# davelee2804/MiMSEM

Hardware: AMD Instinct MI355X
Metric: element operator-applies/sec (higher is better)
Workload: dtype f64; 1 GPU; Umat (B1) matrix-free apply, p=3 24x24x6 cubed sphere x 30 levels (BASELINE config 4 grid); order=3, elements=3456, levels=30, patches_per_gpu=24, form=wave-level fused (k_apply_wave + k_wave_perim)

## Files before the change

include/mimsem_hip.h:

```cpp
#ifndef MIMSEM_HIP_H
#define MIMSEM_HIP_H

#ifdef __cplusplus
extern "C" {
#endif

#define MIMSEM_ABI_VERSION 1

enum {
    MIMSEM_OK = 0,
    MIMSEM_ERR_ARG = -1,
    MIMSEM_ERR_UNSUPPORTED = -2,
    MIMSEM_ERR_HIP = -3,
    MIMSEM_ERR_STATE = -4,
    MIMSEM_ERR_SINGULAR = -5
};

typedef struct mimsem_ctx mimsem_ctx;

typedef struct mimsem_mesh_desc {
    int elOrd;
    int quadOrd;
    int nEl;
    int nk;
// ... 46 lines not shown
const char* mimsem_strerror(int code);
const char* mimsem_last_hip_error(void);
int  mimsem_device_count(void);

int  mimsem_ctx_create(const mimsem_mesh_desc* desc, int device, mimsem_ctx** out);
void mimsem_ctx_destroy(mimsem_ctx* ctx);
int  mimsem_ctx_set_stream(mimsem_ctx* ctx, void* hip_stream);
int  mimsem_ctx_sync(mimsem_ctx* ctx);
int  mimsem_ctx_set_levels(mimsem_ctx* ctx, const double* thick, const double* thickInv);
long long mimsem_ctx_workspace_bytes(const mimsem_ctx* ctx);
int  mimsem_op_level_chunk(const mimsem_ctx* ctx, int nlev);
int  mimsem_op_wave_stats(const mimsem_ctx* ctx, int nlev, int out[5]);
int  mimsem_ctx_set_wave_split(mimsem_ctx* ctx, int part_levels, int order);
int  mimsem_ctx_set_wave_balance(mimsem_ctx* ctx, int ncu, int wgs_per_cu);
long long mimsem_ctx_wave_balance_launches(const mimsem_ctx* ctx);
#define MIMSEM_PART_ALL      0
#define MIMSEM_PART_BOUNDARY 1
#define MIMSEM_PART_INTERIOR 2
int  mimsem_ctx_set_halo_slots(mimsem_ctx* ctx, int form, const int* slots, int n);
int  mimsem_op_apply_part(mimsem_ctx* ctx, int op, int geom_lev0, int nlev, double scale, unsigned flags,
                          const double* f, long long f_stride, const double* x, long long x_stride,
                          double* y, long long y_stride, double alpha, int part);
int  mimsem_op_apply_part_reset(mimsem_ctx* ctx);
int  mimsem_ctx_set_profiling(mimsem_ctx* ctx, int on);
int  mimsem_ctx_profile_read(mimsem_ctx* ctx, double* ms_pass1, double* ms_pass2, long long* launches);

int  mimsem_ctx_use_own_stream(mimsem_ctx* ctx);
int  mimsem_malloc(void** dev, long long bytes);
int  mimsem_free(void* dev);
int  mimsem_memcpy_h2d(mimsem_ctx* ctx, void* dev, const void* host, long long bytes);
// ... 309 lines not shown
```

mimsem_amd/_lib.py:

```python
import ctypes as C
import os
import subprocess

_HERE = os.path.dirname(os.path.abspath(__file__))
LIB_PATH = os.environ.get("MIMSEM_LIB") or os.path.join(_HERE, "libmimsem_hip.so")

c_dp = C.c_void_p
c_ll = C.c_longlong


class MeshDesc(C.Structure):
    _fields_ = [("elOrd", C.c_int), ("quadOrd", C.c_int), ("nEl", C.c_int), ("nk", C.c_int),
                ("n0", C.c_int), ("n1", C.c_int), ("n2", C.c_int),
                ("inds0", C.c_void_p), ("inds1x", C.c_void_p), ("inds1y", C.c_void_p), ("inds2", C.c_void_p),
                ("det", C.c_void_p), ("J", C.c_void_p), ("thick", C.c_void_p), ("thickInv", C.c_void_p),
                ("indsq", C.c_void_p), ("nq", C.c_int)]


class MimsemError(RuntimeError):
    pass


_SIGS = {
    "mimsem_abi_version": (C.c_int, []),
# ... 1 lines not shown
    "mimsem_strerror": (C.c_char_p, [C.c_int]),
    "mimsem_last_hip_error": (C.c_char_p, []),
    "mimsem_device_count": (C.c_int, []),
    "mimsem_ctx_create": (C.c_int, [C.POINTER(MeshDesc), C.c_int, C.POINTER(C.c_void_p)]),
    "mimsem_ctx_destroy": (None, [C.c_void_p]),
    "mimsem_ctx_set_stream": (C.c_int, [C.c_void_p, C.c_void_p]),
    "mimsem_ctx_use_own_stream": (C.c_int, [C.c_void_p]),
    "mimsem_ctx_sync": (C.c_int, [C.c_void_p]),
    "mimsem_ctx_set_levels": (C.c_int, [C.c_void_p, C.c_void_p, C.c_void_p]),
    "mimsem_ctx_workspace_bytes": (c_ll, [C.c_void_p]),
    "mimsem_op_level_chunk": (C.c_int, [C.c_void_p, C.c_int]),
    "mimsem_op_wave_stats": (C.c_int, [C.c_void_p, C.c_int, C.POINTER(C.c_int)]),
    "mimsem_ctx_set_wave_split": (C.c_int, [C.c_void_p, C.c_int, C.c_int]),
    "mimsem_ctx_set_wave_balance": (C.c_int, [C.c_void_p, C.c_int, C.c_int]),
    "mimsem_ctx_wave_balance_launches": (c_ll, [C.c_void_p]),
    "mimsem_ctx_set_halo_slots": (C.c_int, [C.c_void_p, C.c_int, C.c_void_p, C.c_int]),
    "mimsem_op_apply_part": (C.c_int, [C.c_void_p, C.c_int, C.c_int, C.c_int, C.c_double, C.c_uint, c_dp, c_ll, c_dp, c_ll, c_dp, c_ll, C.c_double, C.c_int]),
    "mimsem_ctx_set_profiling": (C.c_int, [C.c_void_p, C.c_int]),
    "mimsem_ctx_profile_read": (C.c_int, [C.c_void_p, C.POINTER(C.c_double), C.POINTER(C.c_double), C.POINTER(c_ll)]),
    "mimsem_malloc": (C.c_int, [C.POINTER(C.c_void_p), c_ll]),
    "mimsem_free": (C.c_int, [C.c_void_p]),
    "mimsem_memcpy_h2d": (C.c_int, [C.c_void_p, C.c_void_p, C.c_void_p, c_ll]),
    "mimsem_memcpy_d2h": (C.c_int, [C.c_void_p, C.c_void_p, C.c_void_p, c_ll]),
    "mimsem_memset": (C.c_int, [C.c_void_p, C.c_void_p, C.c_int, c_ll]),
    "mimsem_op_apply": (C.c_int, [C.c_void_p, C.c_int, C.c_int, C.c_int, C.c_double, C.c_uint,
                                  c_dp, c_ll, c_dp, c_ll, c_dp, c_ll, C.c_double]),
    "mimsem_op_apply_levels": (C.c_int, [C.c_void_p, C.c_int, C.c_int, C.c_int, C.c_int, C.c_double, C.c_uint,
                                         c_dp, c_ll, c_dp, c_ll, c_dp, c_ll, C.c_double]),
    "mimsem_op_apply_up": (C.c_int, [C.c_void_p, C.c_int, C.c_int, C.c_int, C.c_double, C.c_double, C.c_uint,
                                     c_dp, c_ll, c_dp, c_ll, c_dp, c_ll, c_dp, c_ll, C.c_double]),
# ... 184 lines not shown
```

mimsem_amd/csrc/api.hip:

```cpp
#include <algorithm>
#include <cstdio>
#include <cstdlib>
#include <climits>
#include <cstring>
#include "ctx.hpp"
#include "wave_balance.hpp"

namespace mimsem {
thread_local std::string g_last_hip_error;
int hip_fail(hipError_t e, const char* what) {
    g_last_hip_error = std::string(what) + ": " + hipGetErrorString(e);
    return MIMSEM_ERR_HIP;
}
}

namespace {

template <class T>
int upload(T** dst, const T* src, size_t count, mimsem_ctx* c) {
    if (int rc = c->alloc((void**)dst, count*sizeof(T))) return rc;
    if (count) MIMSEM_HIP_TRY(hipMemcpy(*dst, src, count*sizeof(T), hipMemcpyHostToDevice));
    return MIMSEM_OK;
}

// ... 479 lines not shown
        };
        for (int p : owned[g]) {
            ent.push_back(int4{2*p, (int)(contrib(2*p, 0) | contrib(2*p, 1) << 16), (int)(contrib(2*p + 1, 0) | contrib(2*p + 1, 1) << 16), 0});
            W.ndirect += 2;
        }
        if (ent.empty() || ent.size() > 64) return MIMSEM_ERR_UNSUPPORTED;
        for (int t = 0; t < 64; t++) W.plan[(size_t)g*64 + t] = ent[t%ent.size()];
        W.nsides += (int)sides.size(); W.maxsides = std::max(W.maxsides, (int)sides.size());
        if (sides.size() == 4 && nxs > 0 && nys > 0) W.nfull++;
        W.mix[nxs == 2 && nys == 2 ? 0 : (nxs == 4 && nys == 0 ? 1 : (nxs == 0 && nys == 4 ? 2 : 3))]++;
        W.maxgx = std::max(W.maxgx, 16*(int)sides.size());
    }
    return MIMSEM_OK;
}

int level_chunk(const mimsem_ctx* c, int nlev) {
    const ElemSizes& es = c->es;
    const int epb = 256/(es.mp12 <= 4 ? 4 : (es.mp12 <= 16 ? 16 : (es.mp12 <= 32 ? 32 : 64)));
    const long long blocks1 = ((long long)c->nEl + epb - 1)/epb;
    long long lch = (blocks1*nlev)/(256*6);
    if (lch < 1) lch = 1;
    if (lch > nlev) lch = nlev;
    if (lch > 8) lch = 8;
    if (c->lch_override > 0) lch = std::min(c->lch_override, nlev);
    return (int)std::max(1LL, lch);
}

int wave_level_chunk(const mimsem_ctx* c, int nlev) {
    if (c->wave_lch > 0) return std::max(1, std::min(std::min(c->wave_lch, 8), nlev));
    return std::max(1, std::min(8, nlev));
// ... 158 lines not shown
    const bool own = want_own && build_wave_own(es.n, c->n1, c->nEl, es.n1e, 64/lpe, c->h_i1x.data(), c->h_i1y.data(), P, W) == MIMSEM_OK;
    WaveTables t;
    const size_t mark = c->owned.size();
    rc = [&]() -> int {
        int rc;
        if ((rc = upload(&t.lane, P.lane.data(), P.lane.size(), c))) return rc;
        if ((rc = upload(&t.plan, P.plan.data(), P.plan.size(), c))) return rc;
        std::vector<int4> rec(P.pslot.size());
        for (size_t i = 0; i < rec.size(); i++) rec[i] = int4{P.pslot[i], P.ppart[2*i], P.ppart[2*i + 1], 0};
        if ((rc = upload(&t.prec, rec.data(), rec.size(), c))) return rc;
        if ((rc = upload(&t.node, P.node.data(), P.node.size(), c))) return rc;
        if (own) {
            if ((rc = upload(&t.oplan, W.plan.data(), W.plan.size(), c))) return rc;
            if ((rc = upload(&t.gh, W.gh.data(), W.gh.size(), c))) return rc;
            if ((rc = upload(&t.gx, W.gx.data(), W.gx.size(), c))) return rc;
            if (own4 && (rc = upload(&t.gh4, W.gh4.data(), W.gh4.size(), c))) return rc;
        }
        if (P.nsing && (rc = upload(&t.sing, P.sing.data(), P.sing.size(), c))) return rc;
        if ((rc = upload(&t.fin, P.fin.data(), P.fin.size(), c))) return rc;
        if ((rc = upload(&t.sslot, P.sslot.data(), P.sslot.size(), c))) return rc;
        if (P.ntiles > 0 && (rc = upload(&t.tfin, P.tfin.data(), P.tfin.size(), c))) return rc;
        const size_t n = (size_t)std::max(P.nsides, 1)*(size_t)std::max(c->nk, 1);
        if ((rc = c->alloc((void**)&t.cnt, n*sizeof(int)))) return rc;
        MIMSEM_HIP_TRY(hipMemset(t.cnt, 0, n*sizeof(int)));
        std::vector<double> G, Rv;
        pack_wave_metric(c, P, lpe, G, Rv);
        if ((rc = upload(&t.G, G.data(), G.size(), c))) return rc;
        return upload(&t.R, Rv.data(), Rv.size(), c);
    }();
    if (rc) { while (c->owned.size() > mark) c->release(c->owned.back().first); return rc; }
    t.on = true; t.own = own; t.can_fin = P.fin_ok && want_fin; t.split = marked != nullptr;
    t.ndirect = P.ndirect; t.ngroups = P.ngroups; t.nsing = P.nsing; t.nps = P.nps; t.npart = P.npart; t.npwritten = P.npwritten; t.nsides = P.nsides;
    if (P.ntiles > 0) { t.ntiles = P.ntiles; t.ninner = P.ninner; }
    t.nbgroups = P.nbgroups; t.nbrec = P.nbrec;
    c->wv = t;
    if (const char* kind = exp_env("MIMSEM_WPART_MEM")) c->w_partmem = !strcmp(kind, "plain") ? 2 : (!strcmp(kind, "finegrained") ? 1 : 0);
    if (const char* ev = exp_env("MIMSEM_WAVE_ORDER")) c->wave_order = atoi(ev);
    if (const char* ev = exp_env("MIMSEM_WAVE_LCH")) c->wave_lch = atoi(ev);
    if (const char* ev = exp_env("MIMSEM_WAVE_CPP")) c->wave_cpp = atoi(ev);
    if (const char* ev = exp_env("MIMSEM_WAVE2")) c->wave2_mode = atoi(ev);
    if (getenv("MIMSEM_VERBOSE"))
        fprintf(stderr, "[mimsem] wave plan: %d groups of %d elements (%d on the halo boundary), %d perimeter slots (%d partials in %d sides) of %d; "
// ... 288 lines not shown
    if (g->g) (void)hipGraphDestroy(g->g);
    delete g;
}
int mimsem_ctx_sync(mimsem_ctx* c) { if (!c) return MIMSEM_ERR_ARG; MIMSEM_HIP_TRY(hipStreamSynchronize(c->stream)); return MIMSEM_OK; }
long long mimsem_ctx_workspace_bytes(const mimsem_ctx* c) { return c ? c->bytes : 0; }
int mimsem_op_level_chunk(const mimsem_ctx* c, int nlev) { return (c && nlev > 0) ? level_chunk(c, nlev) : MIMSEM_ERR_ARG; }
int mimsem_op_wave_stats(const mimsem_ctx* c, int nlev, int out[5]) {
    if (!c || !out || nlev < 1) return MIMSEM_ERR_ARG;
    for (int i = 0; i < 5; i++) out[i] = 0;
    if (!c->wv.on) return 0;
    out[0] = c->wv.ngroups; out[1] = c->wv.ndirect; out[2] = c->wv.npwritten; out[3] = c->wv.nps;
    if (c->wv.own) { out[1] = c->n1; out[2] = 0; out[3] = 0; }
    if (c->wv.own && c->es.n == 3 && c->wv.ntiles == 0 && !c->d_tIn) {
        const WaveParts wp = wave_level_parts(c, nlev, c->wv.ngroups);
        out[4] = wp.longest;
        const int nwg = c->wv.gh4 ? wave_balance_workgroups(c, nlev, c->wv.ngroups, wp) : 0;
        const mimsem_ctx::BalList* b = nwg > 0 ? wave_balance_find(c, nlev, c->wv.ngroups, nwg) : nullptr;
        if (b && b->items) out[4] = b->longest;
    }
    else { const int lch = wave_level_chunk(c, nlev); out[4] = lch*wave_chunks_per_item(c, nlev, lch, c->wv.ngroups); }
    return 1;
}

int mimsem_ctx_set_wave_split(mimsem_ctx* c, int part_levels, int order) {
    if (!c || part_levels < 0 || order < -1 || order > 3) return MIMSEM_ERR_ARG;
    if (c->is_capturing()) return MIMSEM_ERR_STATE;
    c->wave_part = part_levels;
    if (order >= 0) c->wave_order = order;
    return MIMSEM_OK;
}

int mimsem_ctx_set_wave_balance(mimsem_ctx* c, int ncu, int wgs_per_cu) {
    if (!c || ncu > (1 << 20) || (ncu >= 0 && (wgs_per_cu < 1 || wgs_per_cu > 3))) return MIMSEM_ERR_ARG;
    if (c->is_capturing()) return MIMSEM_ERR_STATE;
    c->bal_ncu = ncu < 0 ? -1 : ncu;
    if (ncu >= 0) c->bal_k = wgs_per_cu;
    return MIMSEM_OK;
}
long long mimsem_ctx_wave_balance_launches(const mimsem_ctx* c) { return c ? c->bal_launches : MIMSEM_ERR_ARG; }

int mimsem_ctx_set_levels(mimsem_ctx* c, const double* thick, const double* thickInv) {
    if (!c) return MIMSEM_ERR_ARG;
    if (c->is_capturing()) return MIMSEM_ERR_STATE;
    MIMSEM_HIP_TRY(hipStreamSynchronize(c->stream));
    const size_t cnt = (size_t)c->nk*c->nEl*c->es.mp12;
    std::vector<double> th(cnt, 1.0), ti(cnt, 1.0);
    if (thick) std::memcpy(th.data(), thick, cnt*sizeof(double));
    if (thickInv) std::memcpy(ti.data(), thickInv, cnt*sizeof(double));
    else if (thick) for (size_t i = 0; i < cnt; i++) ti[i] = 1.0/th[i];
    else if (false) {}
    if (cnt) {
        MIMSEM_HIP_TRY(hipMemcpy(c->d_th, th.data(), cnt*sizeof(double), hipMemcpyHostToDevice));
        MIMSEM_HIP_TRY(hipMemcpy(c->d_tI, ti.data(), cnt*sizeof(double), hipMemcpyHostToDevice));
    }
// ... 169 lines not shown
    return a;
}
static void basis_by_value(const mimsem_ctx* c, ElemArgs& a) {
    for (size_t k = 0; k < 20; k++) a.Etab[k] = k < c->tab.E.size() ? c->tab.E[k] : 0.0;
    for (size_t k = 0; k < 5; k++) a.Wq[k] = k < c->tab.quad.w.size() ? c->tab.quad.w[k] : 0.0;
}
static bool fits_32bit(const mimsem_ctx* c, bool nodes) {
    const long long lim = 1LL << 28;
    return (long long)c->n1 < lim && (!nodes || (long long)c->n0 < lim) && (long long)c->n2 < lim && (long long)c->nEl*c->es.mp12 < lim;
}

#ifdef MIMSEM_STAMPS
static long long* g_stamps = nullptr; static size_t g_stamp_items = 0;
static size_t stamps_begin(mimsem_ctx* c, int nlev, ElemArgs& a) {
    const size_t items = (size_t)c->wv.ngroups*std::max((nlev + a.lch - 1)/a.lch, a.wnp);
    if (!exp_env("MIMSEM_WAVE_STAMPS")) return items;
    if (items > g_stamp_items) { if (g_stamps) (void)hipFree(g_stamps); (void)hipMalloc((void**)&g_stamps, items*16*8); g_stamp_items = items; }
    (void)hipMemsetAsync(g_stamps, 0, items*16*8, c->stream);
    a.wstamps = g_stamps;
    return items;
}
static void stamps_report(mimsem_ctx* c, const ElemArgs& a, size_t items) {
    if (!a.wstamps) return;
    (void)hipStreamSynchronize(c->stream);
    std::vector<long long> h(items*16);
    (void)hipMemcpy(h.data(), g_stamps, items*16*8, hipMemcpyDeviceToHost);
    long long t0 = h[0], t1 = 0;
    for (size_t i = 0; i < items; i++) { t0 = std::min(t0, h[i*16]); t1 = std::max(t1, h[i*16 + 15]); }
    fprintf(stderr, "[stamps] items %zu lch %d  first entry -> last done: %lld ticks\n", items, a.lch, t1 - t0);
    const char* names[16] = {"entry(rel. first)", "barrier", "tables requested", "level loads issued", "batch0", "batch1", "batch2", "batch3",
                             "b4", "b5", "b6", "chunks done", "fin: stores acked", "fin: arrival counted", "fin: sides finished", "stores acked"};
    for (int k = 0; k < 16; k++) {
        std::vector<long long> v;
        for (size_t i = 0; i < items; i++) if (h[i*16 + k]) v.push_back(k == 0 ? h[i*16] - t0 : h[i*16 + k] - h[i*16]);
        if (v.empty()) continue;
        std::sort(v.begin(), v.end());
        fprintf(stderr, "[stamps] %-20s min %8lld  p10 %8lld  median %8lld  p90 %8lld  max %8lld   (ticks since the wave's entry)\n", names[k],
                v.front(), v[v.size()/10], v[v.size()/2], v[v.size()*9/10], v.back());
    }
}
#endif


static int apply_wave2(mimsem_ctx* c, const ApplyCall& k, ElemArgs& a) {
    if (int rc = c->ensure_ye(64)) return rc;
    a.wlane = c->wv.lane; a.wgroups = c->wv.ngroups; a.wG = c->wv.G; a.wR = c->wv.R;
// ... 26 lines not shown
    const int rc = launch_elem_apply(c, k.op, a);
    return rc ? rc : launch_gather_perim(c, k.nlev, c->d_ye, c->f_npart, a.accum, k.y, k.ys);
}

static int apply_wave1(mimsem_ctx* c, const ApplyCall& k, ElemArgs& a, bool splits) {
    const WaveTables& w = c->wv;
    const ElemSizes& es = c->es;
    const int nlev = k.nlev;
    const bool own = w.own && !splits && k.op == MIMSEM_OP_UMAT && es.n == 3 && !c->d_tIn && w.ntiles == 0;
    const long long prow = (own ? 0LL : (long long)w.npart) + 128;
    int g0 = 0, g1 = w.ngroups, r0 = 0, r1 = w.nps;
    if (splits && k.part == MIMSEM_PART_BOUNDARY) { g1 = w.nbgroups; r1 = w.nbrec; }
    if (splits && k.part == MIMSEM_PART_INTERIOR) { g0 = w.nbgroups; r0 = w.nbrec; }
    a.wlane = w.lane; a.wplan = own ? w.oplan : w.plan; a.wgroups = g1 - g0; a.wg0 = g0; a.wdump = own ? 0 : w.npart;
    a.wgh = own ? w.gh : nullptr; a.wgx = w.gx;
    a.wgh4 = (own && (long long)c->nEl*es.mp12 < (1LL << 27)) ? w.gh4 : nullptr;
    a.wsing = w.nsing ? w.sing : nullptr; a.wnode = w.node; a.wG = w.G; a.wR = w.R;
    if (c->d_tIn) { a.tIp = c->d_tIn; a.tps = (long long)c->n0*2; a.tnode = 1; }
    a.lch = wave_level_chunk(c, nlev);
    a.wcpp = wave_chunks_per_item(c, nlev, a.lch, g1 - g0);
    if (own) {
        const WaveParts wp = wave_level_parts(c, nlev, g1 - g0);
        a.wnp = wp.np; a.wpb = wp.pb; a.wpr = wp.pr;
        a.lch = nlev == 1 ? 1 : 8; a.wcpp = 1;
        if (const int nwg = a.wgh4 ? wave_balance_workgroups(c, nlev, g1 - g0, wp) : 0) {
            const mimsem_ctx::BalList* b = wave_balance_find(c, nlev, g1 - g0, nwg);
            if (!b && !c->is_capturing()) {
                if (int rc = wave_balance_make(c, nlev, g1 - g0, nwg, wp)) return rc;
                b = &c->bal.back();
            }
            if (b && b->items) { a.witems = b->items; a.wnitems = b->nitems; }
        }
    }
    a.swz = c->wave_order;
    if (w.ntiles > 0) {
        if (splits) return MIMSEM_ERR_STATE;
        a.wtfin = w.tfin; a.wtile = WTF;
        a.wcpp = std::min(a.wcpp, MIMSEM_WTLEV/8);
        a.swz &= ~2;
// ... 434 lines not shown
```

mimsem_amd/csrc/ctx.hpp:

```cpp
#pragma once
#include <hip/hip_runtime.h>
#include <string>
#include <utility>
#include <vector>
#include "../../include/mimsem_hip.h"
#include "basis_host.hpp"
#include <cstdlib>

constexpr int MIMSEM_RD_COUNTERS = 8;
#ifdef MIMSEM_WITH_EXPERIMENTS
constexpr bool kExperiments = true;
inline const char* exp_env(const char* name) {
    static const bool on = std::getenv("MIMSEM_EXPERIMENTS") && std::atoi(std::getenv("MIMSEM_EXPERIMENTS")) != 0;
    return on ? std::getenv(name) : nullptr;
}
#else
constexpr bool kExperiments = false;
inline const char* exp_env(const char*) { return nullptr; }
#endif

namespace mimsem {
extern thread_local std::string g_last_hip_error;
int hip_fail(hipError_t e, const char* what);
}
// ... 12 lines not shown
struct WaveTables {
    bool on = false;
    int ngroups = 0, nsing = 0, nps = 0, npart = 0, ndirect = 0;
    int npwritten = 0;
    bool can_fin = false;
    int nsides = 0;
    int4* fin = nullptr;
    int* sslot = nullptr;
    int* cnt = nullptr;
    int nbgroups = 0, nbrec = 0; bool split = false;
    int4* lane = nullptr;
    bool own = false;
    int4* oplan = nullptr;
    int4* gh = nullptr;
    int* gx = nullptr;
    int4* gh4 = nullptr;
    int4* tfin = nullptr; int ntiles = 0, ninner = 0;
    int4* plan = nullptr;
    int2* sing = nullptr;
    int* node = nullptr;
    double* G = nullptr;
    double* R = nullptr;
    int4* prec = nullptr;
};

enum class Mem { Plain, Uncached, FineGrained };

struct mimsem_ctx {
    int device = 0;
    hipStream_t stream = nullptr;
    hipStream_t cap_stream = nullptr, cap_saved = nullptr; bool cap_active = false, cap_swapped = false;
// ... 170 lines not shown
};
struct PairBlocks { int nEl, lch; const int *i1x, *i1y, *plan; const double *B, *ye; long long yes; const double* b; double* ze; long long zes; const int4* bplan; };
struct PairGather { const double* ye; long long yes; const int* plan; int nslots; GatherEpilogue g; double* x; };
int launch_sw_pair(mimsem_ctx* c, int PA, int PB, const ElemArgs& ea, const PairBlocks& ba, const PairGather& ga, const ElemArgs& eq, const PairGather& gq);
int launch_gather_epilogue(mimsem_ctx* c, int form, int nlev, const double* ye, long long ye_stride, const GatherEpilogue& g,
                           double* x, long long xs);
int launch_blocks_residual(mimsem_ctx* c, int nlev, const double* B, const double* ye, long long yes,
                           const double* b, long long bs, double* ze, long long zes,
                           const double* escale = nullptr, long long ess = 0);
int launch_elem_apply(mimsem_ctx* c, int op, const ElemArgs& a);
int launch_elem_apply_pending(mimsem_ctx* c, const ElemArgs& a, const ElemPending& pd);
int launch_gather_perim(mimsem_ctx* c, int nlev, const double* yp, long long yps, int accum, double* y, long long ys,
                        const int* pslot = nullptr, const int* ppart = nullptr, int nps = -1);
int launch_apply_wave(mimsem_ctx* c, int op, const ElemArgs& a);
int wave_workgroup_waves();
int launch_apply_wave2(mimsem_ctx* c, int op, const ElemArgs& a);
int launch_wave_perim(mimsem_ctx* c, int nlev, const double* yp, long long yps, int accum, double* y, long long ys, int r0 = 0, int r1 = -1);
int launch_gather_sum(mimsem_ctx* c, int form, int nlev, const double* ye, long long ye_stride, int accum,
                      double* y, long long ys, bool shared_only = false);
int launch_blocks_apply(mimsem_ctx* c, int form, int nlev, int transposed, const double* B, long long bstride_lev,
                        const double* x, long long xs, double* y, long long ys, double alpha, int accum,
                        const double* escale = nullptr, long long escale_stride = 0);
int launch_halo_segments(mimsem_ctx* c, const int* idx, int nseg, const int* seg_off, int s_begin, int s_end, int nlev, int mode,
                         double* buf, double* v, long long vs);
int launch_elmats(mimsem_ctx* c, int op, int lev, double scale, unsigned flags, const double* f, double* out,
                  const double* f2 = nullptr, double param = 0.0);
int launch_incidence(mimsem_ctx* c, int which, int nlev, const double* x, long long xs, double* y, long long ys);
int launch_interp_quad(mimsem_ctx* c, int form, int global, int nlev, const double* x, long long xs, double* out, long long os);
int launch_sw_operator(mimsem_ctx* c, int nlev, double a, double grav, double H, const double* f0, long long f0s,
                       const double* x, long long xs, double* y, long long ys);
// ... 18 lines not shown
```

mimsem_amd/csrc/elem_kernels.hip:

```cpp
#include <hip/hip_ext.h>
#include "ctx.hpp"

namespace {

template <int N> struct Dims {
    static constexpr int n = N, np1 = N + 1, mp1 = N + 1, mp12 = mp1*mp1;
    static constexpr int n0e = np1*np1, n1e = np1*N, n2e = N*N;
    static constexpr int LPE = (mp12 <= 4) ? 4 : (mp12 <= 16 ? 16 : (mp12 <= 32 ? 32 : 64));
    static constexpr int BLOCK = 256, EPB = BLOCK/LPE;
};

enum Space { S0 = 0, S1 = 1, S2 = 2, SN = 3, SQ = 4, SQ2 = 5 };

template <int OP> struct OpTraits;
#define MIMSEM_TRAIT(op, in_, cf_, out_) \
    template <> struct OpTraits<op> { static constexpr Space in = in_, cf = cf_, out = out_; \
         \
        static constexpr int tup = (op == MIMSEM_OP_UMAT_UP) ? 1 : (op == MIMSEM_OP_UVEC_HU_UP ? 2 : (op == MIMSEM_OP_UHMAT_UP ? 3 : 0)); \
        static constexpr bool up = (op == MIMSEM_OP_PHMAT_UP || op == MIMSEM_OP_ROTMAT_UP) || tup != 0; \
         \
         \
        static constexpr bool hs = (op == MIMSEM_OP_UMAT_RAY || op == MIMSEM_OP_UMAT_FRIC); \
        static constexpr Space cf2 = up ? S1 : (hs ? S2 : SN); }
MIMSEM_TRAIT(MIMSEM_OP_UMAT,    S1, SN, S1);
// ... 1505 lines not shown

int launch_gather_perim(mimsem_ctx* c, int nlev, const double* yp, long long yps, int accum, double* y, long long ys,
                        const int* pslot, const int* ppart, int nps) {
    if (nps < 0) { pslot = c->d_pslot; ppart = c->d_ppart; nps = c->f_nps; }
    if (nps == 0 || nlev == 0) return MIMSEM_OK;
    const dim3 grid((unsigned)((nps + 255)/256), (unsigned)((nlev + GS_LC - 1)/GS_LC));
    if (c->ev_k2[0]) hipExtLaunchKernelGGL(k_gather_perim, grid, dim3(256), 0, c->stream, c->ev_k2[0], c->ev_k2[1], 0,
                                           yp, yps, pslot, ppart, nps, nlev, accum, y, ys);
    else hipLaunchKernelGGL(k_gather_perim, grid, dim3(256), 0, c->stream, yp, yps, pslot, ppart, nps, nlev, accum, y, ys);
    c->mark_k2();
    MIMSEM_HIP_TRY(hipGetLastError());
    return MIMSEM_OK;
}

int wave_workgroup_waves() { return WNW; }
template <int N>
static int dispatch_apply_wave(mimsem_ctx* c, int op, const ElemArgs& a) {
    const int nch = (a.nlev + a.lch - 1)/a.lch;
    if (a.wnp > 0 && !a.witems && (a.wtfin || a.wfin || a.wpb < 1 || a.wpr < 0 || a.wpr >= a.wnp || 2*(a.wnp*a.wpb + a.wpr) < a.nlev)) return MIMSEM_ERR_ARG;
    const bool listed = a.witems != nullptr;
    if (listed && (a.wnitems < 1 || !a.wgh || !a.wgh4 || a.lch != WLC || a.wg0 != 0 || N != 3 || MIMSEM_WLB != 2 || MIMSEM_WAHEAD != 2)) return MIMSEM_ERR_ARG;
    const long long items = listed ? (long long)a.wnitems : (long long)a.wgroups*(a.wnp > 0 ? a.wnp : (nch + a.wcpp - 1)/a.wcpp);
    if (items >= (1LL << 31)) return MIMSEM_ERR_UNSUPPORTED;
    const unsigned grid = (unsigned)((items + WNW - 1)/WNW);
    if (grid == 0) return MIMSEM_OK;
    constexpr bool TILEABLE = kExperiments && (N == 3 || N == 4) && WNW == 4;
    const bool tile = a.wtfin != nullptr;
    if (tile && (!TILEABLE || a.wgroups%4 != 0 || a.wg0 != 0 || a.lch*a.wcpp > MIMSEM_WTLEV)) return MIMSEM_ERR_STATE;
    const bool own = a.wgh != nullptr;
    if (own && (N != 3 || op != MIMSEM_OP_UMAT || tile || a.wnp < 1)) return MIMSEM_ERR_STATE;
// ... 465 lines not shown
```

mimsem_amd/csrc/elem_wave.inc:

```
#ifndef MIMSEM_WNW
#define MIMSEM_WNW 4
#endif
#ifndef MIMSEM_WAHEAD
#define MIMSEM_WAHEAD 2
#endif
#ifndef MIMSEM_WLB
#define MIMSEM_WLB 2
#endif
constexpr int WNW = MIMSEM_WNW;
constexpr int WLC = 8;

typedef __attribute__((address_space(1))) double gdouble;
typedef __attribute__((address_space(1))) char gchar;

__device__ __forceinline__ void wave_fence() {
    __builtin_amdgcn_fence(__ATOMIC_RELEASE, "wavefront");
    __builtin_amdgcn_wave_barrier();
    __builtin_amdgcn_fence(__ATOMIC_ACQUIRE, "wavefront");
}

__device__ __forceinline__ void wave_exit_if_done(int left) {
    asm volatile("s_cmp_gt_i32 %0, 0\n\ts_cbranch_scc1 .Lwave_goes_on%=\n\ts_endpgm\n.Lwave_goes_on%=:" :: "s"(left) : "scc", "memory");
}

// ... 33 lines not shown
}

#ifndef MIMSEM_WAVE_NT
#define MIMSEM_WAVE_NT 0
#endif
typedef double wave_d2 __attribute__((ext_vector_type(2)));
#if MIMSEM_WAVE_NT
__device__ __forceinline__ double2 wload2(const void* p) { const wave_d2 v = __builtin_nontemporal_load((const wave_d2*)p); double2 r; r.x = v.x; r.y = v.y; return r; }
#else
__device__ __forceinline__ double2 wload2(const void* p) { return *(const double2*)p; }
#endif
#define WLOAD(T, p) wload2(p)

#ifdef MIMSEM_STAMPS
#define WSTAMP(k) do { if (a.wstamps && lane == 0) a.wstamps[(size_t)item*16 + (k)] = (long long)__builtin_amdgcn_s_memtime(); } while (0)
#else
#define WSTAMP(k) do { } while (0)
#endif

template <int N, int OP, int LCT, bool ACCUM, bool TILE = false, bool OWN = false>
__global__ __launch_bounds__(64*WNW) __attribute__((amdgpu_waves_per_eu(OWN ? 3 : (OpTraits<OP>::cf == SN ? 4 : 3), 8))) void k_apply_wave(ElemArgs a) {
    using D = Dims<N>;
    using T = OpTraits<OP>;
    static_assert(T::in == S1 && T::out == S1 && !T::up && T::cf2 == SN, "1-form -> 1-form operators without upwinding");
    constexpr int LPE = D::LPE, EPW = 64/LPE, ND = 2*D::n1e, NW = WNW;
    constexpr int NACC = EPW*ND, ZERO = NACC + 128;
    constexpr int RS = D::mp1 + (D::mp1 & 1);
    constexpr int XT = D::n1e + D::mp1*RS;
    constexpr int SXE = XT + 2*(LPE - D::n1e) + ((XT + 2*(LPE - D::n1e)) & 1);
    constexpr int WGR = NACC + 136;
    constexpr int SW = (EPW*SXE > WGR + (OWN ? 32 : 0)) ? EPW*SXE : WGR + (OWN ? 32 : 0);
    constexpr int LB = LCT >= MIMSEM_WLB ? MIMSEM_WLB : (LCT >= 2 ? 2 : LCT);
// ... 399 lines not shown
    unsigned g;
    int lbeg, lend_;
    if constexpr (LIST) {
        typedef const __attribute__((address_space(4))) int cint;
        cint* const it = (cint*)(unsigned long long)(wit + item);
        g = (unsigned)it[0]; lbeg = it[1]; lend_ = it[2];
    } else {
        unsigned ch;
        if (a.swz & 2) { g = item/nchunk; ch = item%nchunk; }
        else           { g = item%(unsigned)a.wgroups; ch = item/(unsigned)a.wgroups; }
        g += (unsigned)a.wg0;
        lbeg = 2*((int)ch*a.wpb + min((int)ch, a.wpr));
        lend_ = min(a.nlev, lbeg + 2*(a.wpb + ((int)ch < a.wpr ? 1 : 0)));
    }
    const int lend = lend_;
    const int4 wl = a.wlane[(size_t)g*64 + lane];
    const int4 wp = a.wplan[(size_t)g*64 + lane];
    const int4 gh = a.wgh4[(size_t)g*64 + lane];
    const int gxs = a.wgx[(size_t)g*64 + lane];
    const double2* hp = (const double2*)(a.wG + (size_t)gh.x*4);
    const double2 h01 = hp[0], h23 = hp[1];
    const bool gyn = (gh.z & 1) != 0, gsz = (gh.z & 4) != 0, gidle = (gh.z & 8) != 0;
    const int gc0 = (gh.z & 2) ? 3 : 0;
    const int gm = gyn ? (lane >> 2) & 3 : lane & 3;
    const unsigned gxo = 8u*(unsigned)gxs;
    const unsigned tgo = 16u*(unsigned)gh.y + 8u*(unsigned)(gm & 1), ghi = gm >= 2 ? 0xFFFFFFFFu : 0u;
    const double2* gp = (const double2*)(a.wG + ((size_t)g*64 + lane)*4);
    const double2 g01 = gp[0], g23 = gp[1];
    const double gaa = a.scale*g01.x, gab = a.scale*g01.y, gbb = a.scale*g23.x;
    const int e = wl.x;
    const int qx = q%D::mp1, qy = q/D::mp1;
    const unsigned gq = (unsigned)e*D::mp12 + (unsigned)q;
    const unsigned xo = 8u*(unsigned)wl.y;
    const unsigned to = 16u*gq;
    double2 px[LCT]; double pt0[LCT], pg[LCT], ptg[LCT/(2*LB)];
    auto load_batch = [&](int r0, int lev0_) {
        {
            const int L = a.lev0 + min(lev0_, a.nlev - 1);
            const char* row = (const char*)(a.tIp + ((size_t)(L & 1)*a.tnp + (size_t)(L >> 1))*(size_t)a.tps);
            const double2 tp = WLOAD(double2, row + to);
            pt0[r0] = tp.x; pt0[r0 + 1] = tp.y;
            if ((r0/LB)%2 == 0) {
                const unsigned nx = lev0_ + 2 <= a.nlev - 1 ? 8u*(unsigned)a.tps : 0u;
                ptg[r0/(2*LB)] = *(const double*)(row + (tgo + (ghi & nx)));
            }
        }
#pragma unroll
        for (int i = 0; i < LB; i++) {
            const int r = r0 + i;
            const int lev = min(lev0_ + i, a.nlev - 1);
            px[r] = WLOAD(double2, (const char*)(a.x + (size_t)lev*a.xs) + xo);
            pg[r] = *(const double*)((const char*)(a.x + (size_t)lev*a.xs) + gxo);
        }
    };
#pragma unroll
    for (int b = 0; b < AHEAD; b++) { load_batch(b*LB, lbeg + b*LB); __builtin_amdgcn_sched_barrier(0); }
    {
        double* se = sE[wv];
#pragma unroll
        for (int k = 0; k < D::mp1*N; k++) se[k] = a.Etab[k];
    }
    wave_fence();

    const bool vert = (a.flags & MIMSEM_FLAG_VERT) != 0;
    double Ex[N];
#pragma unroll
    for (int j = 0; j < N; j++) Ex[j] = sE[wv][qx*N + j];
    double cu[4], cp[4], pq[4];
#pragma unroll
    for (int k = 0; k < 4; k++) {
        const int j = (qy - k) & 3;
        cu[k] = j < 3 ? sE[wv][qy*N + j] : 0.0;
        cp[k] = qy < 3 ? a.alpha*sE[wv][j*N + qy] : 0.0;
        pq[k] = qx < 3 ? a.alpha*sE[wv][k*N + qx] : 0.0;
    }
    double kc[3];
    const double hgaa = a.scale*h01.x, hgab = a.scale*h01.y, hgbb = a.scale*h23.x;
    const double gm0 = gyn ? hgab : hgaa, gm1 = gyn ? hgbb : hgab;
#pragma unroll
    for (int t = 0; t < 3; t++) {
        const int tt = !gyn ? t : (gc0 == 0 ? (t == 0 ? 0 : 3 - t) : 2 - t);
        kc[t] = sE[wv][gc0*N + tt];
    }
    const double* const sgl = &s_g[wv][gm][gh.w & 0xFF];
    double* const sdump = &s_x[wv][(lane >> 5) & 1][WGR + 16 + (lane & 15)];
    double* const sgr0 = (!gidle && gm < 2) ? &s_x[wv][gm & 1][WGR + (gh.w >> 8)] : sdump;
    double* const sgr1 = (!gidle && gm >= 2) ? &s_x[wv][gm & 1][WGR + (gh.w >> 8)] : sdump;
    const int xd00 = wl.z & 0xFFFF, xd01 = (wl.z >> 16) & 0xFFFF, xd10 = wl.w & 0xFFFF, xd11 = (wl.w >> 16) & 0xFFFF;
    const bool hasx = q < D::n1e;
    const int aci0 = hasx ? el*ND + q : NACC + lane;
    const int aci1 = qx < 3 ? el*ND + D::n1e + qy*3 + qx : NACC + 64 + lane;
    const int ldx = q < D::n1e ? q : 0, ldy = D::n1e + qy*RS + (qx < 3 ? qx : 0);
    const bool okx = q < D::n1e, oky = qx < 3;
    const int wp00 = wp.y & 0xFFFF, wp01 = (wp.y >> 16) & 0xFFFF, wp10 = wp.z & 0xFFFF, wp11 = (wp.z >> 16) & 0xFFFF;
    const bool wy = wp.x >= 0;
    gchar* wo = (gchar*)(wy ? (a.y + (size_t)lbeg*a.ys + wp.x) : (a.out + (size_t)lbeg*a.os + (-wp.x - 2)));
    const long long wst = 8*(wy ? a.ys : a.os);
#pragma unroll
    for (int i = 0; i < LB; i++) s_x[wv][i][ZERO] = 0.0;
    gchar* const dumpp = (gchar*)(a.out + a.wdump + 2*lane);
    double gkeep = 0.0;
    for (; lbeg < lend; lbeg += LCT) {
    const int nl = lend - lbeg;
#pragma unroll
    for (int b0 = 0; b0 < LCT; b0 += LB) {
        const bool pass = (b0/LB)%2 == 0;
        __builtin_amdgcn_sched_barrier(0);
        load_batch((b0 + AHEAD*LB)%LCT, lbeg + b0 + AHEAD*LB);
        __builtin_amdgcn_sched_barrier(0);
#pragma unroll
        for (int i = 0; i < LB; i++) {
            double* st = s_x[wv][i];
            st[xd00] = px[b0 + i].x; st[xd01] = px[b0 + i].x; st[xd10] = px[b0 + i].y; st[xd11] = px[b0 + i].y;
        }
        if (pass) {
#pragma unroll
            for (int i = 0; i < 2*LB; i++) s_g[wv][i][lane] = pg[b0 + i];
        }
        wave_fence();
        double yxr[LB], yyr[LB];
#pragma unroll
        for (int i = 0; i < LB; i++) {
            const int l = b0 + i;
            const double* sx = s_x[wv][i] + el*SXE;
// ... 21 lines not shown
            gyr = gyn ? Pq : Pr;
        }
        wave_fence();
#pragma unroll
        for (int i = 0; i < LB; i++) { double* sacc = s_x[wv][i]; sacc[aci0] = yxr[i]; sacc[aci1] = yyr[i]; }
        if (pass) { *sgr0 = gyr; gkeep = gyr; }
        else *sgr1 = gkeep;
        wave_fence();
#pragma unroll
        for (int i = 0; i < LB; i++) {
            const int l = b0 + i;
            const double* sacc = s_x[wv][i];
            double2 val;
            val.x = sacc[wp00] + sacc[wp01]; val.y = sacc[wp10] + sacc[wp11];
            gdouble* o = (gdouble*)(l < nl ? wo : dumpp);
            if constexpr (ACCUM) { double o0 = o[0], o1 = o[1]; if (!wy) { o0 = 0.0; o1 = 0.0; } val.x += o0; val.y += o1; }
            o[0] = val.x; o[1] = val.y;
            wo += wst;
        }
        wave_fence();
        if (b0 + LB < LCT) wave_exit_if_done(nl - (b0 + LB));
    }
    }
}
template <int N, int OP, int LCT, bool ACCUM>
__global__ __launch_bounds__(64*WNW) __attribute__((amdgpu_waves_per_eu(3, 8))) void k_apply_wave(ElemArgs a) { apply_wave_body<N, OP, LCT, ACCUM, false>(a); }
template <int N, int OP, int LCT, bool ACCUM>
__global__ __launch_bounds__(64*WNW) __attribute__((amdgpu_waves_per_eu(3, 8))) void k_apply_wave_list(ElemArgs a) { apply_wave_body<N, OP, LCT, ACCUM, true>(a); }
}

template <int OP, int LCT, bool ACCUM>
__global__ __launch_bounds__(64*WNW) __attribute__((amdgpu_waves_per_eu(3, 8))) void k_apply_wave2(ElemArgs a) {
    constexpr int N = 3;
    using D = Dims<N>;
    using T = OpTraits<OP>;
// ... 166 lines not shown
```

Before: 6.803 billion element operator-applies/s.

## Pack per-lane wave tables and metrics into contiguous per-group records

```diff
diff --git a/include/mimsem_hip.h b/include/mimsem_hip.h
--- a/include/mimsem_hip.h
+++ b/include/mimsem_hip.h
@@ -84,6 +84,7 @@
 int  mimsem_ctx_set_wave_split(mimsem_ctx* ctx, int part_levels, int order);
 int  mimsem_ctx_set_wave_balance(mimsem_ctx* ctx, int ncu, int wgs_per_cu);
 long long mimsem_ctx_wave_balance_launches(const mimsem_ctx* ctx);
+int  mimsem_ctx_wave_packed(const mimsem_ctx* ctx);
 #define MIMSEM_PART_ALL      0
 #define MIMSEM_PART_BOUNDARY 1
 #define MIMSEM_PART_INTERIOR 2
diff --git a/mimsem_amd/_lib.py b/mimsem_amd/_lib.py
--- a/mimsem_amd/_lib.py
+++ b/mimsem_amd/_lib.py
@@ -39,6 +39,7 @@
     "mimsem_ctx_set_wave_split": (C.c_int, [C.c_void_p, C.c_int, C.c_int]),
     "mimsem_ctx_set_wave_balance": (C.c_int, [C.c_void_p, C.c_int, C.c_int]),
     "mimsem_ctx_wave_balance_launches": (c_ll, [C.c_void_p]),
+    "mimsem_ctx_wave_packed": (C.c_int, [C.c_void_p]),
     "mimsem_ctx_set_halo_slots": (C.c_int, [C.c_void_p, C.c_int, C.c_void_p, C.c_int]),
     "mimsem_op_apply_part": (C.c_int, [C.c_void_p, C.c_int, C.c_int, C.c_int, C.c_double, C.c_uint, c_dp, c_ll, c_dp, c_ll, c_dp, c_ll, C.c_double, C.c_int]),
     "mimsem_ctx_set_profiling": (C.c_int, [C.c_void_p, C.c_int]),
diff --git a/mimsem_amd/csrc/api.hip b/mimsem_amd/csrc/api.hip
--- a/mimsem_amd/csrc/api.hip
+++ b/mimsem_amd/csrc/api.hip
@@ -5,6 +5,7 @@
 #include <cstring>
 #include "ctx.hpp"
 #include "wave_balance.hpp"
+#include "wave_pack.hpp"
 
 namespace mimsem {
 thread_local std::string g_last_hip_error;
@@ -517,6 +518,35 @@
     return MIMSEM_OK;
 }
 
+bool pack_wave_own4(const WavePlan& P, const WaveOwn& W, const std::vector<double>& G, std::vector<int4>& pk, std::vector<double>& pm) {
+    namespace wp = mimsem::wave_pack;
+    pk.assign((size_t)P.ngroups*128, int4{0, 0, 0, 0});
+    pm.assign((size_t)P.ngroups*wp::METRIC_DOUBLES, 0.0);
+    for (int g = 0; g < P.ngroups; g++)
+        for (int l = 0; l < 64; l++) {
+            const size_t i = (size_t)g*64 + l;
+            const int4 ln = P.lane[i], st = W.plan[i], gh = W.gh4[i];
+            if (ln.x < 0 || ln.y < 0 || st.x < 0 || gh.x < 0 || gh.y < 0 || W.gx[i] < 0 || (gh.w & 3)) return false;
+            wp::Lane r{};
+            r.xslot = (unsigned)ln.y; r.gflags = (unsigned)gh.z; r.dst = (unsigned)st.x; r.gquad = (unsigned)(gh.w & 0xFF)/4;
+            r.elem = (unsigned)ln.x; r.ghpt = (unsigned)gh.y; r.gres = (unsigned)gh.w >> 8; r.gx = (unsigned)W.gx[i];
+            r.xd[0] = ln.z & 0xFFFF; r.xd[1] = (ln.z >> 16) & 0xFFFF; r.xd[2] = ln.w & 0xFFFF; r.xd[3] = (ln.w >> 16) & 0xFFFF;
+            r.wp[0] = st.y & 0xFFFF; r.wp[1] = (st.y >> 16) & 0xFFFF; r.wp[2] = st.z & 0xFFFF; r.wp[3] = (st.z >> 16) & 0xFFFF;
+            if (!wp::fits(r)) return false;
+            const wp::Rec w = wp::pack(r);
+            pk[(size_t)g*128 + l] = int4{(int)w.w[0], (int)w.w[1], (int)w.w[2], (int)w.w[3]};
+            pk[(size_t)g*128 + 64 + l] = int4{(int)w.w[4], (int)w.w[5], (int)w.w[6], (int)w.w[7]};
+            const double* own = &G[i*4];
+            const double* nb = &G[(size_t)gh.x*4];
+            const bool gyn = (gh.z & 1) != 0;
+            double* m = &pm[(size_t)g*wp::METRIC_DOUBLES];
+            m[wp::metric_index(l, 0)] = own[0]; m[wp::metric_index(l, 1)] = own[1]; m[wp::metric_index(l, 2)] = own[2];
+            m[wp::metric_index(l, 3)] = gyn ? nb[1] : nb[0];
+            m[wp::metric_index(l, 4)] = gyn ? nb[2] : nb[1];
+        }
+    return true;
+}
+
 int level_chunk(const mimsem_ctx* c, int nlev) {
     const ElemSizes& es = c->es;
     const int epb = 256/(es.mp12 <= 4 ? 4 : (es.mp12 <= 16 ? 16 : (es.mp12 <= 32 ? 32 : 64)));
@@ -705,7 +735,6 @@
             if ((rc = upload(&t.oplan, W.plan.data(), W.plan.size(), c))) return rc;
             if ((rc = upload(&t.gh, W.gh.data(), W.gh.size(), c))) return rc;
             if ((rc = upload(&t.gx, W.gx.data(), W.gx.size(), c))) return rc;
-            if (own4 && (rc = upload(&t.gh4, W.gh4.data(), W.gh4.size(), c))) return rc;
         }
         if (P.nsing && (rc = upload(&t.sing, P.sing.data(), P.sing.size(), c))) return rc;
         if ((rc = upload(&t.fin, P.fin.data(), P.fin.size(), c))) return rc;
@@ -717,6 +746,13 @@
         std::vector<double> G, Rv;
         pack_wave_metric(c, P, lpe, G, Rv);
         if ((rc = upload(&t.G, G.data(), G.size(), c))) return rc;
+        if (own && own4 && wave_own4_built()) {
+            std::vector<int4> pk; std::vector<double> pm;
+            if (pack_wave_own4(P, W, G, pk, pm)) {
+                if ((rc = upload(&t.pk, pk.data(), pk.size(), c))) return rc;
+                if ((rc = upload(&t.pm, pm.data(), pm.size(), c))) return rc;
+            }
+        }
         return upload(&t.R, Rv.data(), Rv.size(), c);
     }();
     if (rc) { while (c->owned.size() > mark) c->release(c->owned.back().first); return rc; }
@@ -1035,7 +1071,7 @@
     if (c->wv.own && c->es.n == 3 && c->wv.ntiles == 0 && !c->d_tIn) {
         const WaveParts wp = wave_level_parts(c, nlev, c->wv.ngroups);
         out[4] = wp.longest;
-        const int nwg = c->wv.gh4 ? wave_balance_workgroups(c, nlev, c->wv.ngroups, wp) : 0;
+        const int nwg = c->wv.pk ? wave_balance_workgroups(c, nlev, c->wv.ngroups, wp) : 0;
         const mimsem_ctx::BalList* b = nwg > 0 ? wave_balance_find(c, nlev, c->wv.ngroups, nwg) : nullptr;
         if (b && b->items) out[4] = b->longest;
     }
@@ -1059,6 +1095,7 @@
     return MIMSEM_OK;
 }
 long long mimsem_ctx_wave_balance_launches(const mimsem_ctx* c) { return c ? c->bal_launches : MIMSEM_ERR_ARG; }
+int mimsem_ctx_wave_packed(const mimsem_ctx* c) { return c && c->wv.on && c->wv.own && c->wv.pk && c->wv.pm ? 1 : 0; }
 
 int mimsem_ctx_set_levels(mimsem_ctx* c, const double* thick, const double* thickInv) {
     if (!c) return MIMSEM_ERR_ARG;
@@ -1258,7 +1295,7 @@
 static long long* g_stamps = nullptr; static size_t g_stamp_items = 0;
 static size_t stamps_begin(mimsem_ctx* c, int nlev, ElemArgs& a) {
     const size_t items = (size_t)c->wv.ngroups*std::max((nlev + a.lch - 1)/a.lch, a.wnp);
-    if (!exp_env("MIMSEM_WAVE_STAMPS")) return items;
+    if (!getenv("MIMSEM_WAVE_STAMPS")) return items;
     if (items > g_stamp_items) { if (g_stamps) (void)hipFree(g_stamps); (void)hipMalloc((void**)&g_stamps, items*16*8); g_stamp_items = items; }
     (void)hipMemsetAsync(g_stamps, 0, items*16*8, c->stream);
     a.wstamps = g_stamps;
@@ -1272,8 +1309,10 @@
     long long t0 = h[0], t1 = 0;
     for (size_t i = 0; i < items; i++) { t0 = std::min(t0, h[i*16]); t1 = std::max(t1, h[i*16 + 15]); }
     fprintf(stderr, "[stamps] items %zu lch %d  first entry -> last done: %lld ticks\n", items, a.lch, t1 - t0);
+    const bool own4 = a.wgh4 && a.wgh && a.lch == 8;
     const char* names[16] = {"entry(rel. first)", "barrier", "tables requested", "level loads issued", "batch0", "batch1", "batch2", "batch3",
-                             "b4", "b5", "b6", "chunks done", "fin: stores acked", "fin: arrival counted", "fin: sides finished", "stores acked"};
+                             "b4", "b5", "b6", "chunks done", own4 ? "records arrived" : "fin: stores acked", own4 ? "first batch arrived" : "fin: arrival counted",
+                             "fin: sides finished", own4 ? "last stores issued" : "stores acked"};
     for (int k = 0; k < 16; k++) {
         std::vector<long long> v;
         for (size_t i = 0; i < items; i++) if (h[i*16 + k]) v.push_back(k == 0 ? h[i*16] - t0 : h[i*16 + k] - h[i*16]);
@@ -1330,7 +1369,7 @@
     if (splits && k.part == MIMSEM_PART_INTERIOR) { g0 = w.nbgroups; r0 = w.nbrec; }
     a.wlane = w.lane; a.wplan = own ? w.oplan : w.plan; a.wgroups = g1 - g0; a.wg0 = g0; a.wdump = own ? 0 : w.npart;
     a.wgh = own ? w.gh : nullptr; a.wgx = w.gx;
-    a.wgh4 = (own && (long long)c->nEl*es.mp12 < (1LL << 27)) ? w.gh4 : nullptr;
+    a.wgh4 = own ? w.pk : nullptr;
     a.wsing = w.nsing ? w.sing : nullptr; a.wnode = w.node; a.wG = w.G; a.wR = w.R;
     if (c->d_tIn) { a.tIp = c->d_tIn; a.tps = (long long)c->n0*2; a.tnode = 1; }
     a.lch = wave_level_chunk(c, nlev);
@@ -1339,6 +1378,7 @@
         const WaveParts wp = wave_level_parts(c, nlev, g1 - g0);
         a.wnp = wp.np; a.wpb = wp.pb; a.wpr = wp.pr;
         a.lch = nlev == 1 ? 1 : 8; a.wcpp = 1;
+        if (a.wgh4 && a.lch == 8) { a.wlane = w.pk; a.wG = w.pm; }
         if (const int nwg = a.wgh4 ? wave_balance_workgroups(c, nlev, g1 - g0, wp) : 0) {
             const mimsem_ctx::BalList* b = wave_balance_find(c, nlev, g1 - g0, nwg);
             if (!b && !c->is_capturing()) {
diff --git a/mimsem_amd/csrc/ctx.hpp b/mimsem_amd/csrc/ctx.hpp
--- a/mimsem_amd/csrc/ctx.hpp
+++ b/mimsem_amd/csrc/ctx.hpp
@@ -50,7 +50,8 @@
     int4* oplan = nullptr;
     int4* gh = nullptr;
     int* gx = nullptr;
-    int4* gh4 = nullptr;
+    int4* pk = nullptr;
+    double* pm = nullptr;
     int4* tfin = nullptr; int ntiles = 0, ninner = 0;
     int4* plan = nullptr;
     int2* sing = nullptr;
@@ -251,6 +252,7 @@
                         const int* pslot = nullptr, const int* ppart = nullptr, int nps = -1);
 int launch_apply_wave(mimsem_ctx* c, int op, const ElemArgs& a);
 int wave_workgroup_waves();
+bool wave_own4_built();
 int launch_apply_wave2(mimsem_ctx* c, int op, const ElemArgs& a);
 int launch_wave_perim(mimsem_ctx* c, int nlev, const double* yp, long long yps, int accum, double* y, long long ys, int r0 = 0, int r1 = -1);
 int launch_gather_sum(mimsem_ctx* c, int form, int nlev, const double* ye, long long ye_stride, int accum,
diff --git a/mimsem_amd/csrc/elem_kernels.hip b/mimsem_amd/csrc/elem_kernels.hip
--- a/mimsem_amd/csrc/elem_kernels.hip
+++ b/mimsem_amd/csrc/elem_kernels.hip
@@ -1,5 +1,7 @@
 #include <hip/hip_ext.h>
 #include "ctx.hpp"
+#include "wave_pack.hpp"
+namespace wave_pack = mimsem::wave_pack;
 
 namespace {
 
@@ -1543,6 +1545,7 @@
 }
 
 int wave_workgroup_waves() { return WNW; }
+bool wave_own4_built() { return MIMSEM_WLB == 2 && MIMSEM_WAHEAD == 2; }
 template <int N>
 static int dispatch_apply_wave(mimsem_ctx* c, int op, const ElemArgs& a) {
     const int nch = (a.nlev + a.lch - 1)/a.lch;
diff --git a/mimsem_amd/csrc/elem_wave.inc b/mimsem_amd/csrc/elem_wave.inc
--- a/mimsem_amd/csrc/elem_wave.inc
+++ b/mimsem_amd/csrc/elem_wave.inc
@@ -71,8 +71,10 @@
 
 #ifdef MIMSEM_STAMPS
 #define WSTAMP(k) do { if (a.wstamps && lane == 0) a.wstamps[(size_t)item*16 + (k)] = (long long)__builtin_amdgcn_s_memtime(); } while (0)
+#define WSTAMP_ARRIVED(k, v, cond) do { asm volatile("" :: "v"(v) : "memory"); if (cond) WSTAMP(k); } while (0)
 #else
 #define WSTAMP(k) do { } while (0)
+#define WSTAMP_ARRIVED(k, v, cond) do { } while (0)
 #endif
 
 template <int N, int OP, int LCT, bool ACCUM, bool TILE = false, bool OWN = false>
@@ -502,24 +504,22 @@
         lend_ = min(a.nlev, lbeg + 2*(a.wpb + ((int)ch < a.wpr ? 1 : 0)));
     }
     const int lend = lend_;
-    const int4 wl = a.wlane[(size_t)g*64 + lane];
-    const int4 wp = a.wplan[(size_t)g*64 + lane];
-    const int4 gh = a.wgh4[(size_t)g*64 + lane];
-    const int gxs = a.wgx[(size_t)g*64 + lane];
-    const double2* hp = (const double2*)(a.wG + (size_t)gh.x*4);
-    const double2 h01 = hp[0], h23 = hp[1];
-    const bool gyn = (gh.z & 1) != 0, gsz = (gh.z & 4) != 0, gidle = (gh.z & 8) != 0;
-    const int gc0 = (gh.z & 2) ? 3 : 0;
+    WSTAMP(0);
+    const int4* const pk = a.wlane + (size_t)g*128;
+    const int4 pk0 = pk[lane], pk1 = pk[64 + lane];
+    const double* const pm = a.wG + (size_t)g*wave_pack::METRIC_DOUBLES;
+    const double2 g01 = ((const double2*)pm)[lane], g23 = ((const double2*)(pm + 128))[lane];
+    const wave_pack::Lane wl = wave_pack::unpack(wave_pack::Rec{{(unsigned)pk0.x, (unsigned)pk0.y, (unsigned)pk0.z, (unsigned)pk0.w,
+                                                                 (unsigned)pk1.x, (unsigned)pk1.y, (unsigned)pk1.z, (unsigned)pk1.w}});
+    const bool gyn = (wl.gflags & 1) != 0, gsz = (wl.gflags & 4) != 0, gidle = (wl.gflags & 8) != 0;
+    const int gc0 = (wl.gflags & 2) ? 3 : 0;
     const int gm = gyn ? (lane >> 2) & 3 : lane & 3;
-    const unsigned gxo = 8u*(unsigned)gxs;
-    const unsigned tgo = 16u*(unsigned)gh.y + 8u*(unsigned)(gm & 1), ghi = gm >= 2 ? 0xFFFFFFFFu : 0u;
-    const double2* gp = (const double2*)(a.wG + ((size_t)g*64 + lane)*4);
-    const double2 g01 = gp[0], g23 = gp[1];
+    const unsigned gxo = 8u*wl.gx;
+    const unsigned tgo = 16u*wl.ghpt + 8u*(unsigned)(gm & 1), ghi = gm >= 2 ? 0xFFFFFFFFu : 0u;
     const double gaa = a.scale*g01.x, gab = a.scale*g01.y, gbb = a.scale*g23.x;
-    const int e = wl.x;
     const int qx = q%D::mp1, qy = q/D::mp1;
-    const unsigned gq = (unsigned)e*D::mp12 + (unsigned)q;
-    const unsigned xo = 8u*(unsigned)wl.y;
+    const unsigned gq = wl.elem*D::mp12 + (unsigned)q;
+    const unsigned xo = 8u*wl.xslot;
     const unsigned to = 16u*gq;
     double2 px[LCT]; double pt0[LCT], pg[LCT], ptg[LCT/(2*LB)];
     auto load_batch = [&](int r0, int lev0_) {
@@ -541,8 +541,11 @@
             pg[r] = *(const double*)((const char*)(a.x + (size_t)lev*a.xs) + gxo);
         }
     };
+    WSTAMP_ARRIVED(12, xo, true);
 #pragma unroll
     for (int b = 0; b < AHEAD; b++) { load_batch(b*LB, lbeg + b*LB); __builtin_amdgcn_sched_barrier(0); }
+    const double g4 = pm[256 + lane];
+    __builtin_amdgcn_sched_barrier(0);
     {
         double* se = sE[wv];
 #pragma unroll
@@ -563,32 +566,31 @@
         pq[k] = qx < 3 ? a.alpha*sE[wv][k*N + qx] : 0.0;
     }
     double kc[3];
-    const double hgaa = a.scale*h01.x, hgab = a.scale*h01.y, hgbb = a.scale*h23.x;
-    const double gm0 = gyn ? hgab : hgaa, gm1 = gyn ? hgbb : hgab;
+    const double gm0 = a.scale*g23.y, gm1 = a.scale*g4;
 #pragma unroll
     for (int t = 0; t < 3; t++) {
         const int tt = !gyn ? t : (gc0 == 0 ? (t == 0 ? 0 : 3 - t) : 2 - t);
         kc[t] = sE[wv][gc0*N + tt];
     }
-    const double* const sgl = &s_g[wv][gm][gh.w & 0xFF];
+    const double* const sgl = &s_g[wv][gm][4*wl.gquad];
     double* const sdump = &s_x[wv][(lane >> 5) & 1][WGR + 16 + (lane & 15)];
-    double* const sgr0 = (!gidle && gm < 2) ? &s_x[wv][gm & 1][WGR + (gh.w >> 8)] : sdump;
-    double* const sgr1 = (!gidle && gm >= 2) ? &s_x[wv][gm & 1][WGR + (gh.w >> 8)] : sdump;
-    const int xd00 = wl.z & 0xFFFF, xd01 = (wl.z >> 16) & 0xFFFF, xd10 = wl.w & 0xFFFF, xd11 = (wl.w >> 16) & 0xFFFF;
+    double* const sgr0 = (!gidle && gm < 2) ? &s_x[wv][gm & 1][WGR + wl.gres] : sdump;
+    double* const sgr1 = (!gidle && gm >= 2) ? &s_x[wv][gm & 1][WGR + wl.gres] : sdump;
+    const int xd00 = (int)wl.xd[0], xd01 = (int)wl.xd[1], xd10 = (int)wl.xd[2], xd11 = (int)wl.xd[3];
     const bool hasx = q < D::n1e;
     const int aci0 = hasx ? el*ND + q : NACC + lane;
     const int aci1 = qx < 3 ? el*ND + D::n1e + qy*3 + qx : NACC + 64 + lane;
     const int ldx = q < D::n1e ? q : 0, ldy = D::n1e + qy*RS + (qx < 3 ? qx : 0);
     const bool okx = q < D::n1e, oky = qx < 3;
-    const int wp00 = wp.y & 0xFFFF, wp01 = (wp.y >> 16) & 0xFFFF, wp10 = wp.z & 0xFFFF, wp11 = (wp.z >> 16) & 0xFFFF;
-    const bool wy = wp.x >= 0;
-    gchar* wo = (gchar*)(wy ? (a.y + (size_t)lbeg*a.ys + wp.x) : (a.out + (size_t)lbeg*a.os + (-wp.x - 2)));
-    const long long wst = 8*(wy ? a.ys : a.os);
+    const int wp00 = (int)wl.wp[0], wp01 = (int)wl.wp[1], wp10 = (int)wl.wp[2], wp11 = (int)wl.wp[3];
+    gchar* wo = (gchar*)(a.y + (size_t)lbeg*a.ys + wl.dst);
+    const long long wst = 8*a.ys;
 #pragma unroll
     for (int i = 0; i < LB; i++) s_x[wv][i][ZERO] = 0.0;
     gchar* const dumpp = (gchar*)(a.out + a.wdump + 2*lane);
     double gkeep = 0.0;
-    for (; lbeg < lend; lbeg += LCT) {
+    [[maybe_unused]] bool wfirst = true;
+    for (; lbeg < lend; lbeg += LCT, wfirst = false) {
     const int nl = lend - lbeg;
 #pragma unroll
     for (int b0 = 0; b0 < LCT; b0 += LB) {
@@ -596,6 +598,7 @@
         __builtin_amdgcn_sched_barrier(0);
         load_batch((b0 + AHEAD*LB)%LCT, lbeg + b0 + AHEAD*LB);
         __builtin_amdgcn_sched_barrier(0);
+        if (b0 == 0) WSTAMP_ARRIVED(13, px[0].x, wfirst);
 #pragma unroll
         for (int i = 0; i < LB; i++) {
             double* st = s_x[wv][i];
@@ -647,11 +650,12 @@
             double2 val;
             val.x = sacc[wp00] + sacc[wp01]; val.y = sacc[wp10] + sacc[wp11];
             gdouble* o = (gdouble*)(l < nl ? wo : dumpp);
-            if constexpr (ACCUM) { double o0 = o[0], o1 = o[1]; if (!wy) { o0 = 0.0; o1 = 0.0; } val.x += o0; val.y += o1; }
+            if constexpr (ACCUM) { val.x += o[0]; val.y += o[1]; }
             o[0] = val.x; o[1] = val.y;
             wo += wst;
         }
         wave_fence();
+        WSTAMP(15);
         if (b0 + LB < LCT) wave_exit_if_done(nl - (b0 + LB));
     }
     }
diff --git a/mimsem_amd/csrc/wave_pack.hpp b/mimsem_amd/csrc/wave_pack.hpp
--- /dev/null
+++ b/mimsem_amd/csrc/wave_pack.hpp
@@ -0,0 +1,62 @@
+#pragma once
+
+namespace mimsem {
+namespace wave_pack {
+
+struct Lane {
+    unsigned xslot, gflags, dst, gquad, elem, ghpt, gres, gx;
+    unsigned xd[4];
+    unsigned wp[4];
+};
+struct Rec { unsigned w[8]; };
+
+constexpr unsigned BITS_SLOT = 28, BITS_FLAGS = 4, BITS_QUAD = 4, BITS_ELEM = 23, BITS_POS = 9, BITS_GHPT = 27, BITS_RES = 5;
+constexpr unsigned field_max(unsigned bits) { return bits >= 32 ? 0xFFFFFFFFu : (1u << bits) - 1u; }
+constexpr bool field_fits(unsigned v, unsigned bits) { return v <= field_max(bits); }
+
+constexpr bool fits_xslot(unsigned v) { return field_fits(v, BITS_SLOT); }
+constexpr bool fits_dst(unsigned v) { return field_fits(v, BITS_SLOT); }
+constexpr bool fits_gx(unsigned v) { return field_fits(v, BITS_SLOT); }
+constexpr bool fits_gflags(unsigned v) { return field_fits(v, BITS_FLAGS); }
+constexpr bool fits_gquad(unsigned v) { return field_fits(v, BITS_QUAD); }
+constexpr bool fits_elem(unsigned v) { return field_fits(v, BITS_ELEM); }
+constexpr bool fits_ghpt(unsigned v) { return field_fits(v, BITS_GHPT); }
+constexpr bool fits_gres(unsigned v) { return field_fits(v, BITS_RES); }
+constexpr bool fits_pos(unsigned v) { return field_fits(v, BITS_POS); }
+
+constexpr bool fits(const Lane& l) {
+    bool ok = fits_xslot(l.xslot) && fits_gflags(l.gflags) && fits_dst(l.dst) && fits_gquad(l.gquad) && fits_elem(l.elem) &&
+              fits_ghpt(l.ghpt) && fits_gres(l.gres) && fits_gx(l.gx);
+    for (int k = 0; k < 4; k++) ok = ok && fits_pos(l.xd[k]) && fits_pos(l.wp[k]);
+    return ok;
+}
+
+constexpr Rec pack(const Lane& l) {
+    Rec r{};
+    r.w[0] = l.xslot | l.gflags << BITS_SLOT;
+    r.w[1] = l.dst | l.gquad << BITS_SLOT;
+    r.w[2] = l.elem | l.xd[0] << BITS_ELEM;
+    r.w[3] = l.ghpt | l.gres << BITS_GHPT;
+    r.w[4] = l.gx;
+    r.w[5] = l.xd[1] | l.xd[2] << BITS_POS | l.xd[3] << 2*BITS_POS;
+    r.w[6] = l.wp[0] | l.wp[1] << BITS_POS | l.wp[2] << 2*BITS_POS;
+    r.w[7] = l.wp[3];
+    return r;
+}
+constexpr Lane unpack(const Rec& r) {
+    Lane l{};
+    l.xslot = r.w[0] & field_max(BITS_SLOT); l.gflags = r.w[0] >> BITS_SLOT;
+    l.dst = r.w[1] & field_max(BITS_SLOT);   l.gquad = r.w[1] >> BITS_SLOT;
+    l.elem = r.w[2] & field_max(BITS_ELEM);  l.xd[0] = r.w[2] >> BITS_ELEM;
+    l.ghpt = r.w[3] & field_max(BITS_GHPT);  l.gres = r.w[3] >> BITS_GHPT;
+    l.gx = r.w[4] & field_max(BITS_SLOT);
+    l.xd[1] = r.w[5] & field_max(BITS_POS); l.xd[2] = (r.w[5] >> BITS_POS) & field_max(BITS_POS); l.xd[3] = (r.w[5] >> 2*BITS_POS) & field_max(BITS_POS);
+    l.wp[0] = r.w[6] & field_max(BITS_POS); l.wp[1] = (r.w[6] >> BITS_POS) & field_max(BITS_POS); l.wp[2] = (r.w[6] >> 2*BITS_POS) & field_max(BITS_POS);
+    l.wp[3] = r.w[7] & field_max(BITS_POS);
+    return l;
+}
+constexpr unsigned METRIC_DOUBLES = 5*64;
+constexpr unsigned metric_index(unsigned lane, unsigned k) { return k < 4 ? (k/2)*128 + lane*2 + k%2 : 256 + lane; }
+
+}
+}
```

Result: slower. 6.681 billion element operator-applies/s (-1.8%).
